# 0kam/alproj

Hardware: AMD Instinct MI355X
Metric: Gpoints/s projected (pinhole + Brown-Conrady, single pose) over the 100M-vertex DSM; CMA-ES iterations/s in `cma` (higher is better)
Workload: dtype f32

## Files before the change

alproj_amd/csrc/alp_cma.hip:

```cpp
#include "alp_points_internal.h"
#include "alp_sampler.h"

#include <cmath>

namespace {

using namespace alp;

constexpr int CMA_MAX_D = SAMPLER_MAX_D;
constexpr int CMA_MAX_P = 4096;
constexpr int CMA_MAX_STARTS = 1024;
constexpr int64_t CMA_MAX_TOTAL = 65536;
constexpr int TELL_THREADS = 256;
constexpr int JACOBI_MAX_SWEEPS = 40;
constexpr double CMA_EPS = 1e-8;
constexpr double CMA_SIGMA_MAX = 1e32;

struct CmaState {
    double mean[CMA_MAX_D], ps[CMA_MAX_D], pc[CMA_MAX_D], d[CMA_MAX_D];
    double C[CMA_MAX_D * CMA_MAX_D], B[CMA_MAX_D * CMA_MAX_D];
    double BD[CMA_MAX_D * CMA_MAX_D];
    double sigma;
    long long g;
    unsigned k0, k1;
};

struct CmaHyper {
    int D, P, mu, dmax, K;
    double mu_eff, c1, cmu, cc, c_sigma, d_sigma, chi_n, cm, sum_w;
};

struct ExpandArgs {
    double tmpl[ALP_NPARAM];
    double lo[CMA_MAX_D], hi[CMA_MAX_D];
    int idx[CMA_MAX_D];
    double origin[3];
};

template <typename T, int DMAX, bool LF>
__global__ __launch_bounds__(256) void cma_generation_kernel(SamplerArgs a0, ExpandArgs e, const CmaState *__restrict__ states, long long P,
                                                             long long total, double *__restrict__ x_out, double *__restrict__ cand_out,
                                                             PoseRec<T> *__restrict__ recs, long long lf_off) {
    const long long cand = ((long long)blockIdx.x * blockDim.x + threadIdx.x) >> 6;
    if (cand >= total) return;
    const long long start = cand / P, draw = cand - start * P;
    const CmaState *st = states + start;
    const int lane = (int)(threadIdx.x & 63);
    SamplerArgs a = a0;
#pragma unroll
    for (int i = 0; i < DMAX; ++i)
        if (i < a.D) a.mean[i] = st->mean[i];
    a.sigma = st->sigma;
    a.gen = (unsigned)st->g;
    a.k0 = st->k0;
    a.k1 = st->k1;
    const double *BD = st->BD;
    double z[DMAX], x[DMAX];
#pragma unroll
    for (int j = 0; j < DMAX; ++j) z[j] = 0.0;
    int accepted = -1;
    for (int base = 0; base < a.n_max && accepted < 0; base += 64) {
        const int t = base + lane;
        bool ok = false;
        if (t < a.n_max) {
            draw_normals<DMAX>(z, a.D, (unsigned)t, (unsigned)draw, a.gen, a.k0, a.k1);
            ok = make_x<DMAX, false>(a, BD, z, x);
        }
        const unsigned long long m = __ballot(ok);
        if (m) accepted = base + __ffsll((long long)m) - 1;
    }
    const int t_final = accepted >= 0 ? accepted : a.n_max;
    if (lane != (t_final & 63)) return;
    draw_normals<DMAX>(z, a.D, (unsigned)t_final, (unsigned)draw, a.gen, a.k0, a.k1);
    make_x<DMAX, true>(a, BD, z, x);
    double prm[ALP_NPARAM];
    for (int k = 0; k < ALP_NPARAM; ++k) prm[k] = e.tmpl[k];
#pragma unroll
    for (int i = 0; i < DMAX; ++i)
        if (i < a.D) {
            double xi = x[i];
            if (accepted < 0 && a.bounded) xi = fmin(fmax(xi, a.lower[i]), a.upper[i]);
            x_out[cand * a.D + i] = xi;
            prm[e.idx[i]] = xi * (e.hi[i] - e.lo[i]) + e.lo[i];
        }
    for (int k = 0; k < ALP_NPARAM; ++k) cand_out[cand * ALP_NPARAM + k] = prm[k];
    double g[POSE_WORDS];
    fold_pose_hd(prm, e.origin, g);
    for (int k = 0; k < POSE_WORDS; ++k) recs[cand].v[k] = (T)g[k];
    if (LF) {
        double lf[POSE_WORDS];
        lens_free_from_general_hd(g, lf);
        for (int k = 0; k < POSE_WORDS; ++k) recs[lf_off + cand].v[k] = (T)lf[k];
    }
}

__device__ __forceinline__ void circle_pair(int m, int r, int k, int *p, int *q) {
    const int a = k == 0 ? m - 1 : (r + k) % (m - 1);
    const int b = (r - k + (m - 1)) % (m - 1);
    *p = a < b ? a : b;
    *q = a < b ? b : a;
}

__device__ void jacobi_eigen(int D, double *C, double *B, double *d2, double *A, double *A2, double *V, double *V2, double *self_,
                             double *oth, double *dlt, int *partner, int *rotated, int *nrot) {
    const int tid = threadIdx.x;
    const int DD = D * D;
    for (int e = tid; e < DD; e += blockDim.x) {
        const int i = e / D, j = e % D;
        double s = 0;
        for (int k = 0; k < D; ++k) s += B[k * D + i] * B[k * D + j];
        A2[e] = s;
    }
    __syncthreads();
    for (int e = tid; e < DD; e += blockDim.x) {
        const int i = e / D, j = e % D;
        double s = 0;
        for (int k = 0; k < D; ++k) s += B[i * D + k] * ((k == j ? 1.5 : 0.0) - 0.5 * A2[k * D + j]);
        V2[e] = s;
    }
    __syncthreads();
    for (int e = tid; e < DD; e += blockDim.x) B[e] = V2[e];
    __syncthreads();
    for (int e = tid; e < DD; e += blockDim.x) {
        const int i = e / D, j = e % D;
        double s = 0;
        for (int k = 0; k < D; ++k) s += C[i * D + k] * B[k * D + j];
        A2[e] = s;
    }
    __syncthreads();
    for (int e = tid; e < DD; e += blockDim.x) {
        const int i = e / D, j = e % D;
        if (i <= j) {
            double s = 0;
            for (int k = 0; k < D; ++k) s += B[k * D + i] * A2[k * D + j];
            A[i * D + j] = s;
            A[j * D + i] = s;
        }
        V[e] = i == j ? 1.0 : 0.0;
    }
    __syncthreads();
    const int m = (D + 1) & ~1;
    for (int sweep = 0; sweep < JACOBI_MAX_SWEEPS && m >= 2; ++sweep) {
        if (tid == 0) *nrot = 0;
        __syncthreads();
        for (int r = 0; r < m - 1; ++r) {
            if (tid < m / 2) {
                int p, q;
                circle_pair(m, r, tid, &p, &q);
                if (q < D) {
                    const double app = A[p * D + p], aqq = A[q * D + q], apq = A[p * D + q];
                    const double g = 100.0 * fabs(apq);
                    double c = 1.0, s = 0.0, t = 0.0;
                    const bool rot = apq != 0.0 && !(fabs(app) + g == fabs(app) && fabs(aqq) + g == fabs(aqq));
                    if (rot) {
                        const double theta = (aqq - app) / (2.0 * apq);
                        if (fabs(theta) > 1e150) t = 0.5 / theta;
                        else {
                            t = 1.0 / (fabs(theta) + sqrt(theta * theta + 1.0));
                            if (theta < 0) t = -t;
                        }
                        c = 1.0 / sqrt(t * t + 1.0);
                        s = t * c;
                        *nrot = 1;
                    }
                    partner[p] = q; partner[q] = p;
                    self_[p] = c; self_[q] = c;
                    oth[p] = -s; oth[q] = s;
                    dlt[p] = -t * apq; dlt[q] = t * apq;
                    rotated[p] = rotated[q] = rot;
                } else if (p < D) {
                    partner[p] = p; self_[p] = 1.0; oth[p] = 0.0; dlt[p] = 0.0; rotated[p] = 0;
                }
            }
            __syncthreads();
            for (int e = tid; e < DD; e += blockDim.x) {
                const int i = e / D, j = e % D;
                double v;
                if (i == j) v = A[e] + dlt[i];
                else if (partner[i] == j && rotated[i]) v = 0.0;
                else {
                    const int lo = i < j ? i : j, hi = i < j ? j : i;
                    const int plo = partner[lo], phi = partner[hi];
                    v = self_[hi] * A[lo * D + hi];
                    if (oth[hi] != 0.0) v += oth[hi] * A[lo * D + phi];
                    v *= self_[lo];
                    if (oth[lo] != 0.0) {
                        double w = self_[hi] * A[plo * D + hi];
                        if (oth[hi] != 0.0) w += oth[hi] * A[plo * D + phi];
                        v += oth[lo] * w;
                    }
                }
                A2[e] = v;
                double u = V[i * D + j] * self_[j];
                if (oth[j] != 0.0) u += V[i * D + partner[j]] * oth[j];
                V2[e] = u;
            }
            __syncthreads();
            for (int e = tid; e < DD; e += blockDim.x) {
                A[e] = A2[e];
                V[e] = V2[e];
            }
            __syncthreads();
        }
        if (*nrot == 0) break;
        __syncthreads();
    }
    for (int e = tid; e < DD; e += blockDim.x) {
        const int i = e / D, j = e % D;
        double s = 0;
        for (int k = 0; k < D; ++k) s += B[i * D + k] * V[k * D + j];
        V2[e] = s;
    }
    for (int i = tid; i < D; i += blockDim.x) d2[i] = A[i * D + i];
    __syncthreads();
    for (int e = tid; e < DD; e += blockDim.x) B[e] = V2[e];
    __syncthreads();
}

template <bool TELL>
__global__ __launch_bounds__(TELL_THREADS) void cma_tell_kernel(CmaHyper h, CmaState *__restrict__ states, const double *__restrict__ weights,
                                                                const double *__restrict__ X_all, const double *__restrict__ sums_all,
                                                                const double *__restrict__ vals_all, double *__restrict__ loss_all,
                                                                int *__restrict__ order_all, double *__restrict__ ys_all,
                                                                double *__restrict__ wio_all) {
    const long long k = blockIdx.x, kP = k * h.P, kPD = kP * h.D;
    CmaState *__restrict__ st = states + k;
    const double *__restrict__ X = X_all + kPD;
    const double *__restrict__ sums = sums_all ? sums_all + kP : nullptr;
    const double n_total = sums_all ? sums_all[(long long)h.K * h.P] : 0.0;
    const double *__restrict__ vals = vals_all ? vals_all + kP : nullptr;
    double *__restrict__ loss_out = loss_all + kP;
    int *__restrict__ order_out = order_all + kP;
    double *__restrict__ ys = ys_all + kPD;
    double *__restrict__ wio = wio_all + kP;
    constexpr int M = CMA_MAX_D * CMA_MAX_D;
    __shared__ double C[M], B[M], A[M], A2[M], V[M], V2[M];
    __shared__ double mean[CMA_MAX_D], d[CMA_MAX_D], yw[CMA_MAX_D], ps[CMA_MAX_D], pc[CMA_MAX_D], d2[CMA_MAX_D];
    __shared__ double self_[CMA_MAX_D], oth[CMA_MAX_D], dlt[CMA_MAX_D];
    __shared__ int partner[CMA_MAX_D], rotated[CMA_MAX_D];
    __shared__ int nrot;
    __shared__ double sig, hsig;
    const int tid = threadIdx.x, D = h.D, P = h.P, DD = D * D;
    for (int e = tid; e < DD; e += blockDim.x) {
        C[e] = st->C[e];
        B[e] = st->B[e];
    }
    for (int i = tid; i < D; i += blockDim.x) {
        mean[i] = st->mean[i];
        d[i] = st->d[i];
        ps[i] = st->ps[i];
        pc[i] = st->pc[i];
    }
    if (tid == 0) sig = st->sigma;
    __syncthreads();
    if (TELL) {
        const long long g = st->g + 1;
        for (int i = tid; i < P; i += blockDim.x) loss_out[i] = vals ? vals[i] : sums[i] / n_total;
        __syncthreads();
        for (int i = tid; i < P; i += blockDim.x) {
            double ki = loss_out[i];
            if (ki != ki) ki = INFINITY;
            int r = 0;
            for (int j = 0; j < P; ++j) {
                double kj = loss_out[j];
                if (kj != kj) kj = INFINITY;
                r += (kj < ki) || (kj == ki && j < i);
            }
            order_out[r] = i;
        }
        __syncthreads();
        const double sigma = sig;
        for (int e = tid; e < P * D; e += blockDim.x) {
            const int r = e / D, j = e % D;
            ys[e] = (X[(long long)order_out[r] * D + j] - mean[j]) / sigma;
        }
        __syncthreads();
        for (int j = tid; j < D; j += blockDim.x) {
            double s = 0.0;
            for (int r = 0; r < h.mu; ++r) s = s + ys[(long long)r * D + j] * weights[r];
            yw[j] = s;
        }
        __syncthreads();
        const double cs = h.c_sigma, cmsig = h.cm * sigma;
        for (int e = tid; e < DD; e += blockDim.x) {
            const int i = e / D, j = e % D;
            double s = 0.0;
            for (int k = 0; k < D; ++k) s += (B[i * D + k] / d[k]) * B[j * D + k];
            A[e] = s;
        }
        for (int j = tid; j < D; j += blockDim.x) mean[j] = mean[j] + cmsig * yw[j];
        __syncthreads();
        const double sq_ps = sqrt(cs * (2.0 - cs) * h.mu_eff);
        for (int i = tid; i < D; i += blockDim.x) {
            double s = 0.0;
            for (int k = 0; k < D; ++k) s += A[i * D + k] * yw[k];
            ps[i] = (1.0 - cs) * ps[i] + sq_ps * s;
        }
        __syncthreads();
        if (tid == 0) {
            double nn = 0.0;
            for (int k = 0; k < D; ++k) nn += ps[k] * ps[k];
            const double norm_ps = sqrt(nn);
            double s2 = sig * exp((cs / h.d_sigma) * (norm_ps / h.chi_n - 1.0));
            sig = s2 < CMA_SIGMA_MAX ? s2 : CMA_SIGMA_MAX;
            const double h_left = norm_ps / sqrt(1.0 - pow(1.0 - cs, (double)(2 * (g + 1))));
            const double h_right = (1.4 + 2.0 / (double)(D + 1)) * h.chi_n;
            hsig = h_left < h_right ? 1.0 : 0.0;
        }
        __syncthreads();
        const double h_sigma = hsig, cc = h.cc;
        const double sq_pc = h_sigma * sqrt(cc * (2.0 - cc) * h.mu_eff);
        for (int i = tid; i < D; i += blockDim.x) pc[i] = (1.0 - cc) * pc[i] + sq_pc * yw[i];
        for (int r = tid; r < P; r += blockDim.x) {
            const double wr = weights[r];
            if (wr >= 0) {
                wio[r] = wr * 1.0;
            } else {
                double nn = 0.0;
                for (int i = 0; i < D; ++i) {
                    double s = 0.0;
                    for (int k = 0; k < D; ++k) s += ys[(long long)r * D + k] * A[i * D + k];
                    nn += s * s;
                }
                const double nrm = sqrt(nn);
                wio[r] = wr * ((double)D / (nrm * nrm + CMA_EPS));
            }
        }
        __syncthreads();
        const double delta_h = (1.0 - h_sigma) * cc * (2.0 - cc);
        const double c1 = h.c1, cmu = h.cmu;
        const double coef = 1.0 + c1 * delta_h - c1 - cmu * h.sum_w;
        for (int e = tid; e < DD; e += blockDim.x) {
            const int i = e / D, j = e % D;
            double rmu = 0.0;
            for (int r = 0; r < P; ++r) rmu += (ys[(long long)r * D + i] * wio[r]) * ys[(long long)r * D + j];
            A2[e] = coef * C[e] + c1 * (pc[i] * pc[j]) + cmu * rmu;
        }
        __syncthreads();
        for (int e = tid; e < DD; e += blockDim.x) C[e] = A2[e];
        if (tid == 0) st->g = g;
        __syncthreads();
    }
    for (int e = tid; e < DD; e += blockDim.x) {
        const int i = e / D, j = e % D;
        A2[e] = (C[i * D + j] + C[j * D + i]) / 2.0;
    }
    __syncthreads();
    for (int e = tid; e < DD; e += blockDim.x) C[e] = A2[e];
    __syncthreads();
    jacobi_eigen(D, C, B, d2, A, A2, V, V2, self_, oth, dlt, partner, rotated, &nrot);
    for (int i = tid; i < D; i += blockDim.x) d[i] = sqrt(d2[i] < 0 ? CMA_EPS : d2[i]);
    __syncthreads();
    for (int e = tid; e < DD; e += blockDim.x) {
        const int i = e / D, j = e % D;
        double s = 0.0;
        for (int k = 0; k < D; ++k) s += (B[i * D + k] * (d[k] * d[k])) * B[j * D + k];
        st->C[e] = s;
        st->B[e] = B[e];
    }
    for (int e = tid; e < h.dmax * h.dmax; e += blockDim.x) {
        const int i = e / h.dmax, j = e % h.dmax;
        st->BD[e] = (i < D && j < D) ? B[i * D + j] * d[j] : 0.0;
    }
    for (int i = tid; i < D; i += blockDim.x) {
        st->d[i] = d[i];
        if (TELL) {
            st->mean[i] = mean[i];
            st->ps[i] = ps[i];
            st->pc[i] = pc[i];
        }
    }
    if (TELL && tid == 0) st->sigma = sig;
}

}

struct alp_cma {
    alp_points *pts = nullptr;
    CmaHyper hy{};
    SamplerArgs sa{};
    ExpandArgs ex{};
    std::vector<uint64_t> seeds;
    bool lens_free = false, shared_pose = false;
    DeviceBuffer<> dev;
    CmaState *st = nullptr;
    double *w = nullptr, *X = nullptr, *cand = nullptr, *loss = nullptr, *ys = nullptr, *wio = nullptr, *vals = nullptr;
    int *order = nullptr;
    bool pending = false;
    bool have_last = false;
    int64_t rows() const { return (int64_t)hy.K * hy.P; }
};

namespace alp {
void cma_points_gone(alp_cma_t *h) { h->pts = nullptr; }
}

namespace {

void fill_state(const alp_cma *h, int k, CmaState *s, const double *mean, double sigma, const double *C, const double *ps, const double *pc,
                int64_t g) {
    const int D = h->hy.D;
    memset(s, 0, sizeof(*s));
    for (int i = 0; i < D; ++i) {
        s->mean[i] = mean[i];
        s->ps[i] = ps[i];
        s->pc[i] = pc[i];
        s->d[i] = 1.0;
        s->B[i * D + i] = 1.0;
    }
    for (int e = 0; e < D * D; ++e) s->C[e] = C[e];
    s->sigma = sigma;
    s->g = g;
    s->k0 = (unsigned)h->seeds[(size_t)k];
    s->k1 = (unsigned)(h->seeds[(size_t)k] >> 32);
}

int upload_states(alp_cma *h, int k0, int n, const CmaState *s) {
    hipStream_t st = ctx().stream;
    ALP_HIP(hipMemcpyAsync(h->st + k0, s, (size_t)n * sizeof(CmaState), hipMemcpyHostToDevice, st));
    hipLaunchKernelGGL(cma_tell_kernel<false>, dim3(n), dim3(TELL_THREADS), 0, st, h->hy, h->st + k0, (const double *)h->w,
                       (const double *)h->X, (const double *)nullptr, (const double *)nullptr, h->loss, h->order, h->ys, h->wio);
    ALP_HIP(hipGetLastError());
    ALP_HIP(hipStreamSynchronize(st));
    return ALP_OK;
}

int usable(alp_cma *h, const char *what) {
    if (int rc = require_init()) return rc;
    if (!h) return fail(ALP_EINVAL, "%s: handle is NULL", what);
    if (h->pending) return fail(ALP_ESTATE, "%s: generations are enqueued; call alp_cma_wait first", what);
    return ALP_OK;
}

template <typename T, int DMAX>
void launch_generation(alp_cma *h, unsigned grid, hipStream_t st) {
    alp_points *p = h->pts;
    PoseRec<T> *recs = (PoseRec<T> *)p->cand_dev;
    if (h->lens_free)
        hipLaunchKernelGGL((cma_generation_kernel<T, DMAX, true>), dim3(grid), dim3(256), 0, st, h->sa, h->ex, (const CmaState *)h->st,
                           (long long)h->hy.P, (long long)h->rows(), h->X, h->cand, recs, (long long)p->cand_cap);
    else
        hipLaunchKernelGGL((cma_generation_kernel<T, DMAX, false>), dim3(grid), dim3(256), 0, st, h->sa, h->ex, (const CmaState *)h->st,
                           (long long)h->hy.P, (long long)h->rows(), h->X, h->cand, recs, (long long)p->cand_cap);
}

template <typename T>
void launch_generation_t(alp_cma *h, unsigned grid, hipStream_t st) {
    if (h->hy.dmax == 12) launch_generation<T, 12>(h, grid, st);
    else if (h->hy.dmax == 24) launch_generation<T, 24>(h, grid, st);
    else launch_generation<T, 32>(h, grid, st);
}

}

extern "C" {

int alp_cma_create_starts(alp_points_t *pts, const double tmpl[ALP_NPARAM], const int32_t *target_idx, int D, const double *lower,
                          const double *upper, int64_t P, int K, const double *weights, const double hyper[ALP_CMA_NHYPER],
                          int n_max_resampling, const uint64_t *seeds, alp_cma_t **out) {
    if (int rc = require_init()) return rc;
    ALP_REQUIRE(out, "out is NULL");
    *out = nullptr;
    ALP_REQUIRE(pts && tmpl && target_idx && lower && upper && weights && hyper && seeds, "NULL argument");
    ALP_REQUIRE(D >= 1 && D <= CMA_MAX_D, "D must be in [1, 32]");
    ALP_REQUIRE(P >= 1 && P <= CMA_MAX_P, "P must be in [1, 4096]");
    ALP_REQUIRE(K >= 1 && K <= CMA_MAX_STARTS, "K must be in [1, 1024]");
    ALP_REQUIRE((int64_t)K * P <= CMA_MAX_TOTAL, "K * P must be at most 65536");
    ALP_REQUIRE(n_max_resampling >= 0 && n_max_resampling <= (1 << 20), "n_max_resampling out of range");
    if (!pts->uo) return fail(ALP_ESTATE, "alp_cma_create: observed uv not set");
    for (int i = 0; i < D; ++i) {
        ALP_REQUIRE(target_idx[i] >= 0 && target_idx[i] < ALP_NPARAM, "target index out of range");
        ALP_REQUIRE(target_idx[i] != 21 && target_idx[i] != 22, "w and h cannot be targets (every candidate must share the image size)");
    }
    const int mu = (int)hyper[0];
    ALP_REQUIRE(mu >= 0 && mu <= P, "mu out of range");
    alp_cma *h = new alp_cma();
    h->pts = pts;
    const int dmax = D <= 12 ? 12 : (D <= 24 ? 24 : 32);
    h->hy = CmaHyper{D, (int)P, mu, dmax, K, hyper[1], hyper[2], hyper[3], hyper[4], hyper[5], hyper[6], hyper[7], hyper[8], hyper[9]};
    h->seeds.assign(seeds, seeds + K);
    memset(&h->sa, 0, sizeof(h->sa));
    for (int i = 0; i < D; ++i) {
        h->sa.lower[i] = 0.0;
        h->sa.upper[i] = 1.0;
    }
    h->sa.D = D;
    h->sa.n_max = n_max_resampling;
    h->sa.bounded = 1;
    memset(&h->ex, 0, sizeof(h->ex));
    for (int k = 0; k < ALP_NPARAM; ++k) h->ex.tmpl[k] = tmpl[k];
    for (int i = 0; i < D; ++i) {
        h->ex.idx[i] = target_idx[i];
        h->ex.lo[i] = lower[i];
        h->ex.hi[i] = upper[i];
    }
    memcpy(h->ex.origin, pts->origin, sizeof(h->ex.origin));
    bool lf = !getenv("ALP_POP_NO_LENS_FREE");
    for (int k = 9; k <= 20 && lf; ++k) lf = tmpl[k] == 0.0;
    for (int i = 0; i < D && lf; ++i) lf = !(target_idx[i] >= 9 && target_idx[i] <= 20);
    bool shared = P > 1 && !lf;
    for (int i = 0; i < D && shared; ++i) shared = target_idx[i] >= 7 && target_idx[i] <= 20;
    h->lens_free = lf;
    h->shared_pose = shared;
    const int64_t R = (int64_t)K * P;
    const size_t sz_state = round_up((int64_t)K * sizeof(CmaState), 256), sz_w = round_up(P * 8, 256), sz_p = round_up(R * 8, 256),
                 sz_pd = round_up(R * D * 8, 256), sz_cand = round_up(R * ALP_NPARAM * 8, 256), sz_ord = round_up(R * 4, 256);
    int rc = h->dev.reserve(sz_state + sz_w + 3 * sz_p + 2 * sz_pd + sz_cand + sz_ord);
    if (!rc) {
        char *q = (char *)h->dev;
        h->st = (CmaState *)q; q += sz_state;
        h->w = (double *)q; q += sz_w;
        h->loss = (double *)q; q += sz_p;
        h->wio = (double *)q; q += sz_p;
        h->vals = (double *)q; q += sz_p;
        h->X = (double *)q; q += sz_pd;
        h->ys = (double *)q; q += sz_pd;
        h->cand = (double *)q; q += sz_cand;
        h->order = (int *)q;
        if (hipMemcpy(h->w, weights, (size_t)P * 8, hipMemcpyHostToDevice) != hipSuccess) rc = fail(ALP_EHIP, "alp_cma_create: weights upload failed");
    }
    if (!rc) rc = points_pop_reserve(pts, R);
    if (!rc) {
        std::vector<double> mean(D, 0.5), C((size_t)D * D, 0.0), zero(D, 0.0);
        for (int i = 0; i < D; ++i) C[(size_t)i * D + i] = 1.0;
        std::vector<CmaState> s((size_t)K);
        for (int k = 0; k < K; ++k) fill_state(h, k, &s[(size_t)k], mean.data(), 1.0, C.data(), zero.data(), zero.data(), 0);
        rc = upload_states(h, 0, K, s.data());
    }
    if (rc) {
        delete h;
        return rc;
    }
    pts->loops.push_back(h);
    *out = h;
    return ALP_OK;
}

int alp_cma_create(alp_points_t *pts, const double tmpl[ALP_NPARAM], const int32_t *target_idx, int D, const double *lower,
                   const double *upper, int64_t P, const double *weights, const double hyper[ALP_CMA_NHYPER], int n_max_resampling,
                   uint64_t seed, alp_cma_t **out) {
    return alp_cma_create_starts(pts, tmpl, target_idx, D, lower, upper, P, 1, weights, hyper, n_max_resampling, &seed, out);
}

int alp_cma_destroy(alp_cma_t *h) {
    if (!h) return ALP_OK;
    if (ctx().ready) hipStreamSynchronize(ctx().stream);
    if (h->pts) {
        h->pts->loop_pending = false;
        auto &v = h->pts->loops;
        for (size_t i = 0; i < v.size(); ++i)
            if (v[i] == h) {
                v.erase(v.begin() + (long)i);
                break;
            }
    }
    delete h;
    return ALP_OK;
}

int alp_cma_set_state_at(alp_cma_t *h, int k, const double *mean, double sigma, const double *C, const double *p_sigma, const double *pc,
                         int64_t generation) {
    if (int rc = usable(h, "alp_cma_set_state")) return rc;
    ALP_REQUIRE(k >= 0 && k < h->hy.K, "start index out of range");
    ALP_REQUIRE(mean && C && p_sigma && pc, "NULL argument");
    ALP_REQUIRE(sigma > 0, "sigma must be positive");
    ALP_REQUIRE(generation >= 0, "generation is negative");
    CmaState s;
    fill_state(h, k, &s, mean, sigma, C, p_sigma, pc, generation);
    return upload_states(h, k, 1, &s);
}

int alp_cma_set_state(alp_cma_t *h, const double *mean, double sigma, const double *C, const double *p_sigma, const double *pc,
                      int64_t generation) {
    return alp_cma_set_state_at(h, 0, mean, sigma, C, p_sigma, pc, generation);
}

int alp_cma_get_state_at(alp_cma_t *h, int k, double *mean, double *sigma, double *C, double *p_sigma, double *pc, int64_t *generation,
                         double *B, double *Dvec) {
    if (int rc = usable(h, "alp_cma_get_state")) return rc;
    ALP_REQUIRE(k >= 0 && k < h->hy.K, "start index out of range");
    CmaState s;
    ALP_HIP(hipMemcpyAsync(&s, h->st + k, sizeof(s), hipMemcpyDeviceToHost, ctx().stream));
    ALP_HIP(hipStreamSynchronize(ctx().stream));
    const int D = h->hy.D;
    for (int i = 0; i < D; ++i) {
        if (mean) mean[i] = s.mean[i];
        if (p_sigma) p_sigma[i] = s.ps[i];
        if (pc) pc[i] = s.pc[i];
        if (Dvec) Dvec[i] = s.d[i];
    }
    for (int e = 0; e < D * D; ++e) {
        if (C) C[e] = s.C[e];
        if (B) B[e] = s.B[e];
    }
    if (sigma) *sigma = s.sigma;
    if (generation) *generation = s.g;
    return ALP_OK;
}

int alp_cma_get_state(alp_cma_t *h, double *mean, double *sigma, double *C, double *p_sigma, double *pc, int64_t *generation, double *B,
                      double *Dvec) {
    return alp_cma_get_state_at(h, 0, mean, sigma, C, p_sigma, pc, generation, B, Dvec);
}

int alp_cma_run(alp_cma_t *h, int64_t generations, int loss_kind, double f_scale) {
    if (int rc = usable(h, "alp_cma_run")) return rc;
    ALP_REQUIRE(generations >= 0, "generations is negative");
    ALP_REQUIRE(loss_kind == ALP_LOSS_MEAN_DIST || loss_kind == ALP_LOSS_HUBER, "unknown loss_kind");
    alp_points *p = h->pts;
    if (!p) return fail(ALP_ESTATE, "alp_cma_run: the point set of this device loop has been destroyed");
    if (p->pending_P > 0 || p->loop_pending)
        return fail(ALP_ESTATE, "alp_cma_run: the point set has an evaluation enqueued that has not been waited for");
    if (generations == 0) return ALP_OK;
    const int64_t R = h->rows();
    if (int rc = points_pop_reserve(p, R)) return rc;
    const unsigned grid = (unsigned)((R * 64 + 255) / 256);
    const bool batched = h->hy.K > 1;
    hipStream_t st = ctx().stream;
    h->pending = true;
    p->loop_pending = true;
    for (int64_t g = 0; g < generations; ++g) {
        if (p->precision == ALP_F64) launch_generation_t<double>(h, grid, st);
        else launch_generation_t<float>(h, grid, st);
        ALP_HIP(hipGetLastError());
        if (int rc = popeval_launch(p, R, loss_kind, f_scale, h->lens_free, h->shared_pose, batched, h->cand)) return rc;
        hipLaunchKernelGGL(cma_tell_kernel<true>, dim3(h->hy.K), dim3(TELL_THREADS), 0, st, h->hy, h->st, (const double *)h->w,
                           (const double *)h->X, (const double *)p->sums_dev, (const double *)nullptr, h->loss, h->order, h->ys, h->wio);
        ALP_HIP(hipGetLastError());
    }
    h->have_last = true;
    return ALP_OK;
}

int alp_cma_wait(alp_cma_t *h) {
    if (int rc = require_init()) return rc;
    ALP_REQUIRE(h, "handle is NULL");
    if (!h->pending) return fail(ALP_ESTATE, "alp_cma_wait: nothing enqueued");
    h->pending = false;
    if (h->pts) h->pts->loop_pending = false;
    ALP_HIP(hipStreamSynchronize(ctx().stream));
    return ALP_OK;
}

int alp_cma_tell_host(alp_cma_t *h, const double *X, const double *losses, int32_t *order_out) {
    if (int rc = usable(h, "alp_cma_tell_host")) return rc;
    ALP_REQUIRE(X && losses, "NULL argument");
    const int64_t R = h->rows(), D = h->hy.D;
    hipStream_t st = ctx().stream;
    ALP_HIP(hipMemcpyAsync(h->X, X, (size_t)(R * D) * 8, hipMemcpyHostToDevice, st));
    ALP_HIP(hipMemcpyAsync(h->vals, losses, (size_t)R * 8, hipMemcpyHostToDevice, st));
    hipLaunchKernelGGL(cma_tell_kernel<true>, dim3(h->hy.K), dim3(TELL_THREADS), 0, st, h->hy, h->st, (const double *)h->w,
                       (const double *)h->X, (const double *)nullptr, (const double *)h->vals, h->loss, h->order, h->ys, h->wio);
    ALP_HIP(hipGetLastError());
    if (order_out) ALP_HIP(hipMemcpyAsync(order_out, h->order, (size_t)R * 4, hipMemcpyDeviceToHost, st));
    ALP_HIP(hipStreamSynchronize(st));
    h->have_last = false;
    return ALP_OK;
}

int alp_cma_fetch_last(alp_cma_t *h, double *X, double *cand, double *losses) {
    if (int rc = usable(h, "alp_cma_fetch_last")) return rc;
    if (!h->have_last) return fail(ALP_ESTATE, "alp_cma_fetch_last: no device generation has run");
    const int64_t R = h->rows(), D = h->hy.D;
    hipStream_t st = ctx().stream;
    if (X) ALP_HIP(hipMemcpyAsync(X, h->X, (size_t)(R * D) * 8, hipMemcpyDeviceToHost, st));
    if (cand) ALP_HIP(hipMemcpyAsync(cand, h->cand, (size_t)R * ALP_NPARAM * 8, hipMemcpyDeviceToHost, st));
    if (losses) ALP_HIP(hipMemcpyAsync(losses, h->loss, (size_t)R * 8, hipMemcpyDeviceToHost, st));
    ALP_HIP(hipStreamSynchronize(st));
    return ALP_OK;
}

}
```

alproj_amd/csrc/host/alp_fold.h:

```cpp
#pragma once

#include <cmath>

#include "alproj_hip.h"

#if defined(__HIP__)
#define ALP_HD __host__ __device__
#else
#define ALP_HD
#endif

namespace alp {

ALP_HD inline double fold_sin(double a) { return std::sin(a); }
ALP_HD inline double fold_cos(double a) { return std::cos(a); }
ALP_HD inline double fold_tan(double a) { return std::tan(a); }

template <typename T>
ALP_HD inline void fold_pose_any(const T p[ALP_NPARAM], double w, double h, const double origin[3], T rec[POSE_WORDS]) {
    const T X = p[0], Y = p[1], Z = p[2], fov = p[3], pan_d = p[4], tilt_d = p[5],
            roll_d = p[6];
    const T cx = p[23], cy = p[24];
    const double pi = M_PI;

    const T fov_x = fov * pi / 180;
    const T fov_y = fov_x * h / w;
    const T fx = w / (2 * fold_tan(fov_x / 2));
    const T fy = h / (2 * fold_tan(fov_y / 2));

    const T a = pan_d * pi / 180;
    const T b = -(tilt_d + 90) * pi / 180;
    const T c = -roll_d * pi / 180;
    const T rz[3][3] = {{fold_cos(a), -fold_sin(a), 0}, {fold_sin(a), fold_cos(a), 0}, {0, 0, 1}};
    const T rx[3][3] = {{1, 0, 0}, {0, fold_cos(b), -fold_sin(b)}, {0, fold_sin(b), fold_cos(b)}};
    const T ry[3][3] = {{fold_cos(c), 0, fold_sin(c)}, {0, 1, 0}, {-fold_sin(c), 0, fold_cos(c)}};
    T rxy[3][3], R[3][3];
    for (int i = 0; i < 3; ++i)
        for (int j = 0; j < 3; ++j) {
            T s = 0;
            for (int k = 0; k < 3; ++k) s += rx[i][k] * ry[k][j];
            rxy[i][j] = s;
        }
    for (int i = 0; i < 3; ++i)
        for (int j = 0; j < 3; ++j) {
            T s = 0;
            for (int k = 0; k < 3; ++k) s += rxy[i][k] * rz[k][j];
            R[i][j] = s;
        }
    const T d[3] = {origin[0] - X, origin[1] - Y, origin[2] - Z};
    T row[3][4];
    for (int i = 0; i < 3; ++i) {
        for (int j = 0; j < 3; ++j) row[i][j] = R[i][j];
        row[i][3] = R[i][0] * d[0] + R[i][1] * d[1] + R[i][2] * d[2];
    }
    const double c0 = (double)(float)((w - 1) / 2);
    const double c1 = (double)(float)((h - 1) / 2);
    const double A = (w - c0) / c0;
    for (int j = 0; j < 4; ++j) {
        const T rowx = fx * row[0][j] + cx * row[2][j];
        const T rowy = fy * row[1][j] + cy * row[2][j];
        rec[0 + j] = A * row[2][j] - rowx / c0;
        rec[4 + j] = rowy / c1 - row[2][j];
        rec[8 + j] = row[2][j];
    }
    for (int i = 0; i < 6; ++i) rec[12 + i] = p[9 + i];
    rec[18] = 1 + p[7];
    rec[19] = 1 + p[8];
    rec[20] = 2 * p[15];
    rec[21] = 2 * p[16];
    for (int i = 0; i < 4; ++i) rec[22 + i] = p[17 + i];
    rec[26] = c0;
    rec[27] = c1;
    rec[28] = -c0;
    rec[29] = -c1;
    rec[30] = rec[31] = 0;
}

ALP_HD inline void fold_pose_hd(const double p[ALP_NPARAM], const double origin[3], double rec[POSE_WORDS]) {
    fold_pose_any<double>(p, p[21], p[22], origin, rec);
}

ALP_HD inline void lens_free_from_general_hd(const double g[POSE_WORDS], double rec[POSE_WORDS]) {
    const double sy = g[18] / g[19];
    for (int i = 0; i < POSE_WORDS; ++i) rec[i] = 0;
    for (int j = 0; j < 4; ++j) {
        rec[0 + j] = g[28] * g[0 + j];
        rec[4 + j] = (g[29] * sy) * g[4 + j];
        rec[8 + j] = g[8 + j];
    }
    rec[26] = g[26];
    rec[27] = g[27];
}

}
```

Measured before the change: 498.4.

## Parallelize CMA ask/tell: wave-spread trig, per-wave Jacobi rounds, shared-memory small tell

The ask kernel keeps the accepted sample in every lane so it is not redrawn, and spreads the eight pose trig evaluations across lanes with shuffles. The Jacobi eigen solver replaces the block barrier and copy-back with per-wave round buffers, ping-pong buffer swaps and a ballot to detect convergence, and the modulo work in pair selection is removed. A SMALL tell variant stages losses, weights, order and ys in shared memory, and the block size now scales with the problem size. This targets the many serial double-precision steps and barriers per CMA iteration, at the cost of more register pressure and more complex code paths.

```diff
diff --git a/alproj_amd/csrc/alp_cma.hip b/alproj_amd/csrc/alp_cma.hip
--- a/alproj_amd/csrc/alp_cma.hip
+++ b/alproj_amd/csrc/alp_cma.hip
@@ -12,6 +12,7 @@
 constexpr int CMA_MAX_STARTS = 1024;
 constexpr int64_t CMA_MAX_TOTAL = 65536;
 constexpr int TELL_THREADS = 256;
+constexpr int TELL_SMALL_P = 256;
 constexpr int JACOBI_MAX_SWEEPS = 40;
 constexpr double CMA_EPS = 1e-8;
 constexpr double CMA_SIGMA_MAX = 1e32;
@@ -57,22 +58,25 @@
     const double *BD = st->BD;
     double z[DMAX], x[DMAX];
 #pragma unroll
-    for (int j = 0; j < DMAX; ++j) z[j] = 0.0;
+    for (int j = 0; j < DMAX; ++j) z[j] = x[j] = 0.0;
     int accepted = -1;
+    constexpr bool KEEP = DMAX <= 24;
     for (int base = 0; base < a.n_max && accepted < 0; base += 64) {
         const int t = base + lane;
         bool ok = false;
         if (t < a.n_max) {
             draw_normals<DMAX>(z, a.D, (unsigned)t, (unsigned)draw, a.gen, a.k0, a.k1);
-            ok = make_x<DMAX, false>(a, BD, z, x);
+            ok = make_x<DMAX, KEEP>(a, BD, z, x);
         }
         const unsigned long long m = __ballot(ok);
         if (m) accepted = base + __ffsll((long long)m) - 1;
     }
     const int t_final = accepted >= 0 ? accepted : a.n_max;
-    if (lane != (t_final & 63)) return;
-    draw_normals<DMAX>(z, a.D, (unsigned)t_final, (unsigned)draw, a.gen, a.k0, a.k1);
-    make_x<DMAX, true>(a, BD, z, x);
+    const int src = t_final & 63;
+    if ((!KEEP || accepted < 0) && lane == src) {
+        draw_normals<DMAX>(z, a.D, (unsigned)t_final, (unsigned)draw, a.gen, a.k0, a.k1);
+        make_x<DMAX, true>(a, BD, z, x);
+    }
     double prm[ALP_NPARAM];
     for (int k = 0; k < ALP_NPARAM; ++k) prm[k] = e.tmpl[k];
 #pragma unroll
@@ -80,12 +84,29 @@
         if (i < a.D) {
             double xi = x[i];
             if (accepted < 0 && a.bounded) xi = fmin(fmax(xi, a.lower[i]), a.upper[i]);
-            x_out[cand * a.D + i] = xi;
+            if (lane == src) x_out[cand * a.D + i] = xi;
             prm[e.idx[i]] = xi * (e.hi[i] - e.lo[i]) + e.lo[i];
         }
+    double ang[FOLD_ANGLES];
+    FoldTrigValues<double> tr;
+    fold_angles<double>(prm, prm[21], prm[22], ang);
+    double mine = 0.0;
+#pragma unroll
+    for (int k = 0; k < FOLD_ANGLES; ++k) {
+        const double ak = __shfl(ang[k], src);
+        if (fold_trig_angle(lane & 7) == k) mine = ak;
+    }
+    double val = 0.0;
+    if (lane < FOLD_SIN_A) {
+        if (lane < FOLD_COS_A) val = fold_tan(mine);
+        else val = fold_cos(mine);
+    } else if (lane < FOLD_TRIGS) val = fold_sin(mine);
+#pragma unroll
+    for (int v = 0; v < FOLD_TRIGS; ++v) tr.v[v] = __shfl(val, v);
+    if (lane != src) return;
     for (int k = 0; k < ALP_NPARAM; ++k) cand_out[cand * ALP_NPARAM + k] = prm[k];
     double g[POSE_WORDS];
-    fold_pose_hd(prm, e.origin, g);
+    fold_pose_with<double>(prm, prm[21], prm[22], e.origin, tr, g);
     for (int k = 0; k < POSE_WORDS; ++k) recs[cand].v[k] = (T)g[k];
     if (LF) {
         double lf[POSE_WORDS];
@@ -95,43 +116,51 @@
 }
 
 __device__ __forceinline__ void circle_pair(int m, int r, int k, int *p, int *q) {
-    const int a = k == 0 ? m - 1 : (r + k) % (m - 1);
-    const int b = (r - k + (m - 1)) % (m - 1);
+    const int a = k == 0 ? m - 1 : (r + k >= m - 1 ? r + k - (m - 1) : r + k);
+    const int b = r - k < 0 ? r - k + (m - 1) : r - k;
     *p = a < b ? a : b;
     *q = a < b ? b : a;
 }
 
-__device__ void jacobi_eigen(int D, double *C, double *B, double *d2, double *A, double *A2, double *V, double *V2, double *self_,
-                             double *oth, double *dlt, int *partner, int *rotated, int *nrot) {
-    const int tid = threadIdx.x;
+struct JacobiRound {
+    double self_[CMA_MAX_D], oth[CMA_MAX_D], dlt[CMA_MAX_D];
+    int partner[CMA_MAX_D], rotated[CMA_MAX_D];
+};
+
+__device__ void jacobi_eigen(int D, double *C, double *B, double *d2, double *A, double *A2, double *V, double *V2, JacobiRound *rnd) {
+    const int tid = threadIdx.x, nthr = blockDim.x;
     const int DD = D * D;
-    for (int e = tid; e < DD; e += blockDim.x) {
+    for (int e = tid; e < DD; e += nthr) {
         const int i = e / D, j = e % D;
         double s = 0;
+#pragma unroll 4
         for (int k = 0; k < D; ++k) s += B[k * D + i] * B[k * D + j];
         A2[e] = s;
     }
     __syncthreads();
-    for (int e = tid; e < DD; e += blockDim.x) {
+    for (int e = tid; e < DD; e += nthr) {
         const int i = e / D, j = e % D;
         double s = 0;
+#pragma unroll 4
         for (int k = 0; k < D; ++k) s += B[i * D + k] * ((k == j ? 1.5 : 0.0) - 0.5 * A2[k * D + j]);
         V2[e] = s;
     }
     __syncthreads();
-    for (int e = tid; e < DD; e += blockDim.x) B[e] = V2[e];
-    __syncthreads();
-    for (int e = tid; e < DD; e += blockDim.x) {
+    for (int e = tid; e < DD; e += nthr) B[e] = V2[e];
+    __syncthreads();
+    for (int e = tid; e < DD; e += nthr) {
         const int i = e / D, j = e % D;
         double s = 0;
+#pragma unroll 4
         for (int k = 0; k < D; ++k) s += C[i * D + k] * B[k * D + j];
         A2[e] = s;
     }
     __syncthreads();
-    for (int e = tid; e < DD; e += blockDim.x) {
+    for (int e = tid; e < DD; e += nthr) {
         const int i = e / D, j = e % D;
         if (i <= j) {
             double s = 0;
+#pragma unroll 4
             for (int k = 0; k < D; ++k) s += B[k * D + i] * A2[k * D + j];
             A[i * D + j] = s;
             A[j * D + i] = s;
@@ -140,13 +169,16 @@
     }
     __syncthreads();
     const int m = (D + 1) & ~1;
+    const int lane = tid & 63;
+    JacobiRound &w = rnd[tid >> 6];
+    const int i0 = tid / D, j0 = tid % D, istep = nthr / D, jstep = nthr % D;
     for (int sweep = 0; sweep < JACOBI_MAX_SWEEPS && m >= 2; ++sweep) {
-        if (tid == 0) *nrot = 0;
-        __syncthreads();
+        int any = 0;
         for (int r = 0; r < m - 1; ++r) {
-            if (tid < m / 2) {
+            int rot_here = 0;
+            if (lane < m / 2) {
                 int p, q;
-                circle_pair(m, r, tid, &p, &q);
+                circle_pair(m, r, lane, &p, &q);
                 if (q < D) {
                     const double app = A[p * D + p], aqq = A[q * D + q], apq = A[p * D + q];
                     const double g = 100.0 * fabs(apq);
@@ -161,63 +193,64 @@
                         }
                         c = 1.0 / sqrt(t * t + 1.0);
                         s = t * c;
-                        *nrot = 1;
+                        rot_here = 1;
                     }
-                    partner[p] = q; partner[q] = p;
-                    self_[p] = c; self_[q] = c;
-                    oth[p] = -s; oth[q] = s;
-                    dlt[p] = -t * apq; dlt[q] = t * apq;
-                    rotated[p] = rotated[q] = rot;
+                    w.partner[p] = q; w.partner[q] = p;
+                    w.self_[p] = c; w.self_[q] = c;
+                    w.oth[p] = -s; w.oth[q] = s;
+                    w.dlt[p] = -t * apq; w.dlt[q] = t * apq;
+                    w.rotated[p] = w.rotated[q] = rot;
                 } else if (p < D) {
-                    partner[p] = p; self_[p] = 1.0; oth[p] = 0.0; dlt[p] = 0.0; rotated[p] = 0;
+                    w.partner[p] = p; w.self_[p] = 1.0; w.oth[p] = 0.0; w.dlt[p] = 0.0; w.rotated[p] = 0;
                 }
             }
+            __builtin_amdgcn_wave_barrier();
+            int i = i0, j = j0;
+            for (int e = tid; e < DD; e += nthr) {
+                const int pi = w.partner[i], pj = w.partner[j], roti = w.rotated[i];
+                const double ci = w.self_[i], cj = w.self_[j], oi = w.oth[i], oj = w.oth[j], di = w.dlt[i];
+                const bool up = i < j;
+                const int lo = up ? i : j, hi = up ? j : i, plo = up ? pi : pj, phi = up ? pj : pi;
+                const double clo = up ? ci : cj, chi = up ? cj : ci, olo = up ? oi : oj, ohi = up ? oj : oi;
+                const double a_e = A[e], a_lh = A[lo * D + hi], a_lp = A[lo * D + phi], a_ph = A[plo * D + hi], a_pp = A[plo * D + phi];
+                const double v_ij = V[i * D + j], v_ip = V[i * D + pj];
+                double v = chi * a_lh;
+                v = ohi != 0.0 ? v + ohi * a_lp : v;
+                v *= clo;
+                double t = chi * a_ph;
+                t = ohi != 0.0 ? t + ohi * a_pp : t;
+                v = olo != 0.0 ? v + olo * t : v;
+                v = (pi == j && roti) ? 0.0 : v;
+                v = i == j ? a_e + di : v;
+                A2[e] = v;
+                double u = v_ij * cj;
+                u = oj != 0.0 ? u + v_ip * oj : u;
+                V2[e] = u;
+                i += istep;
+                j += jstep;
+                if (j >= D) { j -= D; ++i; }
+            }
+            any |= __ballot(rot_here) != 0;
             __syncthreads();
-            for (int e = tid; e < DD; e += blockDim.x) {
-                const int i = e / D, j = e % D;
-                double v;
-                if (i == j) v = A[e] + dlt[i];
-                else if (partner[i] == j && rotated[i]) v = 0.0;
-                else {
-                    const int lo = i < j ? i : j, hi = i < j ? j : i;
-                    const int plo = partner[lo], phi = partner[hi];
-                    v = self_[hi] * A[lo * D + hi];
-                    if (oth[hi] != 0.0) v += oth[hi] * A[lo * D + phi];
-                    v *= self_[lo];
-                    if (oth[lo] != 0.0) {
-                        double w = self_[hi] * A[plo * D + hi];
-                        if (oth[hi] != 0.0) w += oth[hi] * A[plo * D + phi];
-                        v += oth[lo] * w;
-                    }
-                }
-                A2[e] = v;
-                double u = V[i * D + j] * self_[j];
-                if (oth[j] != 0.0) u += V[i * D + partner[j]] * oth[j];
-                V2[e] = u;
-            }
-            __syncthreads();
-            for (int e = tid; e < DD; e += blockDim.x) {
-                A[e] = A2[e];
-                V[e] = V2[e];
-            }
-            __syncthreads();
-        }
-        if (*nrot == 0) break;
-        __syncthreads();
-    }
-    for (int e = tid; e < DD; e += blockDim.x) {
+            double *sw = A; A = A2; A2 = sw;
+            sw = V; V = V2; V2 = sw;
+        }
+        if (!any) break;
+    }
+    for (int e = tid; e < DD; e += nthr) {
         const int i = e / D, j = e % D;
         double s = 0;
+#pragma unroll 4
         for (int k = 0; k < D; ++k) s += B[i * D + k] * V[k * D + j];
         V2[e] = s;
     }
-    for (int i = tid; i < D; i += blockDim.x) d2[i] = A[i * D + i];
-    __syncthreads();
-    for (int e = tid; e < DD; e += blockDim.x) B[e] = V2[e];
-    __syncthreads();
-}
-
-template <bool TELL>
+    for (int i = tid; i < D; i += nthr) d2[i] = A[i * D + i];
+    __syncthreads();
+    for (int e = tid; e < DD; e += nthr) B[e] = V2[e];
+    __syncthreads();
+}
+
+template <bool TELL, bool SMALL = false>
 __global__ __launch_bounds__(TELL_THREADS) void cma_tell_kernel(CmaHyper h, CmaState *__restrict__ states, const double *__restrict__ weights,
                                                                 const double *__restrict__ X_all, const double *__restrict__ sums_all,
                                                                 const double *__restrict__ vals_all, double *__restrict__ loss_all,
@@ -231,14 +264,15 @@
     const double *__restrict__ vals = vals_all ? vals_all + kP : nullptr;
     double *__restrict__ loss_out = loss_all + kP;
     int *__restrict__ order_out = order_all + kP;
-    double *__restrict__ ys = ys_all + kPD;
-    double *__restrict__ wio = wio_all + kP;
     constexpr int M = CMA_MAX_D * CMA_MAX_D;
     __shared__ double C[M], B[M], A[M], A2[M], V[M], V2[M];
+    double *const ys = SMALL ? V : ys_all + kPD;
+    double *const loss = SMALL ? V2 : loss_out;
+    double *const wio = SMALL ? V2 + TELL_SMALL_P : wio_all + kP;
+    const double *const wts = SMALL ? V2 + 2 * TELL_SMALL_P : weights;
+    int *const order = SMALL ? (int *)(V2 + 3 * TELL_SMALL_P) : order_out;
     __shared__ double mean[CMA_MAX_D], d[CMA_MAX_D], yw[CMA_MAX_D], ps[CMA_MAX_D], pc[CMA_MAX_D], d2[CMA_MAX_D];
-    __shared__ double self_[CMA_MAX_D], oth[CMA_MAX_D], dlt[CMA_MAX_D];
-    __shared__ int partner[CMA_MAX_D], rotated[CMA_MAX_D];
-    __shared__ int nrot;
+    __shared__ JacobiRound rnd[TELL_THREADS / 64];
     __shared__ double sig, hsig;
     const int tid = threadIdx.x, D = h.D, P = h.P, DD = D * D;
     for (int e = tid; e < DD; e += blockDim.x) {
@@ -255,29 +289,39 @@
     __syncthreads();
     if (TELL) {
         const long long g = st->g + 1;
-        for (int i = tid; i < P; i += blockDim.x) loss_out[i] = vals ? vals[i] : sums[i] / n_total;
-        __syncthreads();
         for (int i = tid; i < P; i += blockDim.x) {
-            double ki = loss_out[i];
+            const double l = vals ? vals[i] : sums[i] / n_total;
+            loss_out[i] = l;
+            if (SMALL) {
+                loss[i] = l;
+                V2[2 * TELL_SMALL_P + i] = weights[i];
+            }
+        }
+        __syncthreads();
+        for (int i = tid; i < P; i += blockDim.x) {
+            double ki = loss[i];
             if (ki != ki) ki = INFINITY;
             int r = 0;
+#pragma unroll 4
             for (int j = 0; j < P; ++j) {
-                double kj = loss_out[j];
+                double kj = loss[j];
                 if (kj != kj) kj = INFINITY;
                 r += (kj < ki) || (kj == ki && j < i);
             }
             order_out[r] = i;
+            if (SMALL) order[r] = i;
         }
         __syncthreads();
         const double sigma = sig;
         for (int e = tid; e < P * D; e += blockDim.x) {
             const int r = e / D, j = e % D;
-            ys[e] = (X[(long long)order_out[r] * D + j] - mean[j]) / sigma;
+            ys[e] = (X[(long long)order[r] * D + j] - mean[j]) / sigma;
         }
         __syncthreads();
         for (int j = tid; j < D; j += blockDim.x) {
             double s = 0.0;
-            for (int r = 0; r < h.mu; ++r) s = s + ys[(long long)r * D + j] * weights[r];
+#pragma unroll 4
+            for (int r = 0; r < h.mu; ++r) s = s + ys[(long long)r * D + j] * wts[r];
             yw[j] = s;
         }
         __syncthreads();
@@ -285,6 +329,7 @@
         for (int e = tid; e < DD; e += blockDim.x) {
             const int i = e / D, j = e % D;
             double s = 0.0;
+#pragma unroll 4
             for (int k = 0; k < D; ++k) s += (B[i * D + k] / d[k]) * B[j * D + k];
             A[e] = s;
         }
@@ -293,6 +338,7 @@
         const double sq_ps = sqrt(cs * (2.0 - cs) * h.mu_eff);
         for (int i = tid; i < D; i += blockDim.x) {
             double s = 0.0;
+#pragma unroll 4
             for (int k = 0; k < D; ++k) s += A[i * D + k] * yw[k];
             ps[i] = (1.0 - cs) * ps[i] + sq_ps * s;
         }
@@ -312,13 +358,14 @@
         const double sq_pc = h_sigma * sqrt(cc * (2.0 - cc) * h.mu_eff);
         for (int i = tid; i < D; i += blockDim.x) pc[i] = (1.0 - cc) * pc[i] + sq_pc * yw[i];
         for (int r = tid; r < P; r += blockDim.x) {
-            const double wr = weights[r];
+            const double wr = wts[r];
             if (wr >= 0) {
                 wio[r] = wr * 1.0;
             } else {
                 double nn = 0.0;
                 for (int i = 0; i < D; ++i) {
                     double s = 0.0;
+#pragma unroll 4
                     for (int k = 0; k < D; ++k) s += ys[(long long)r * D + k] * A[i * D + k];
                     nn += s * s;
                 }
@@ -333,6 +380,7 @@
         for (int e = tid; e < DD; e += blockDim.x) {
             const int i = e / D, j = e % D;
             double rmu = 0.0;
+#pragma unroll 4
             for (int r = 0; r < P; ++r) rmu += (ys[(long long)r * D + i] * wio[r]) * ys[(long long)r * D + j];
             A2[e] = coef * C[e] + c1 * (pc[i] * pc[j]) + cmu * rmu;
         }
@@ -348,12 +396,13 @@
     __syncthreads();
     for (int e = tid; e < DD; e += blockDim.x) C[e] = A2[e];
     __syncthreads();
-    jacobi_eigen(D, C, B, d2, A, A2, V, V2, self_, oth, dlt, partner, rotated, &nrot);
+    jacobi_eigen(D, C, B, d2, A, A2, V, V2, rnd);
     for (int i = tid; i < D; i += blockDim.x) d[i] = sqrt(d2[i] < 0 ? CMA_EPS : d2[i]);
     __syncthreads();
     for (int e = tid; e < DD; e += blockDim.x) {
         const int i = e / D, j = e % D;
         double s = 0.0;
+#pragma unroll 4
         for (int k = 0; k < D; ++k) s += (B[i * D + k] * (d[k] * d[k])) * B[j * D + k];
         st->C[e] = s;
         st->B[e] = B[e];
@@ -371,6 +420,20 @@
         }
     }
     if (TELL && tid == 0) st->sigma = sig;
+}
+
+int tell_threads(const CmaHyper &h) {
+    const int want = h.D * h.D > h.P ? h.D * h.D : h.P;
+    const int waves = (want + 63) / 64;
+    return 64 * (waves < 1 ? 1 : waves > TELL_THREADS / 64 ? TELL_THREADS / 64 : waves);
+}
+
+bool tell_small(const CmaHyper &h) { return h.P <= TELL_SMALL_P && h.P * h.D <= CMA_MAX_D * CMA_MAX_D; }
+
+template <typename... Args>
+void launch_tell(const CmaHyper &hy, hipStream_t st, Args... args) {
+    if (tell_small(hy)) hipLaunchKernelGGL((cma_tell_kernel<true, true>), dim3(hy.K), dim3(tell_threads(hy)), 0, st, hy, args...);
+    else hipLaunchKernelGGL((cma_tell_kernel<true, false>), dim3(hy.K), dim3(tell_threads(hy)), 0, st, hy, args...);
 }
 
 }
@@ -418,7 +481,7 @@
 int upload_states(alp_cma *h, int k0, int n, const CmaState *s) {
     hipStream_t st = ctx().stream;
     ALP_HIP(hipMemcpyAsync(h->st + k0, s, (size_t)n * sizeof(CmaState), hipMemcpyHostToDevice, st));
-    hipLaunchKernelGGL(cma_tell_kernel<false>, dim3(n), dim3(TELL_THREADS), 0, st, h->hy, h->st + k0, (const double *)h->w,
+    hipLaunchKernelGGL(cma_tell_kernel<false>, dim3(n), dim3(tell_threads(h->hy)), 0, st, h->hy, h->st + k0, (const double *)h->w,
                        (const double *)h->X, (const double *)nullptr, (const double *)nullptr, h->loss, h->order, h->ys, h->wio);
     ALP_HIP(hipGetLastError());
     ALP_HIP(hipStreamSynchronize(st));
@@ -624,8 +687,8 @@
         else launch_generation_t<float>(h, grid, st);
         ALP_HIP(hipGetLastError());
         if (int rc = popeval_launch(p, R, loss_kind, f_scale, h->lens_free, h->shared_pose, batched, h->cand)) return rc;
-        hipLaunchKernelGGL(cma_tell_kernel<true>, dim3(h->hy.K), dim3(TELL_THREADS), 0, st, h->hy, h->st, (const double *)h->w,
-                           (const double *)h->X, (const double *)p->sums_dev, (const double *)nullptr, h->loss, h->order, h->ys, h->wio);
+        launch_tell(h->hy, st, h->st, (const double *)h->w, (const double *)h->X, (const double *)p->sums_dev, (const double *)nullptr,
+                    h->loss, h->order, h->ys, h->wio);
         ALP_HIP(hipGetLastError());
     }
     h->have_last = true;
@@ -649,8 +712,8 @@
     hipStream_t st = ctx().stream;
     ALP_HIP(hipMemcpyAsync(h->X, X, (size_t)(R * D) * 8, hipMemcpyHostToDevice, st));
     ALP_HIP(hipMemcpyAsync(h->vals, losses, (size_t)R * 8, hipMemcpyHostToDevice, st));
-    hipLaunchKernelGGL(cma_tell_kernel<true>, dim3(h->hy.K), dim3(TELL_THREADS), 0, st, h->hy, h->st, (const double *)h->w,
-                       (const double *)h->X, (const double *)nullptr, (const double *)h->vals, h->loss, h->order, h->ys, h->wio);
+    launch_tell(h->hy, st, h->st, (const double *)h->w, (const double *)h->X, (const double *)nullptr, (const double *)h->vals, h->loss,
+                h->order, h->ys, h->wio);
     ALP_HIP(hipGetLastError());
     if (order_out) ALP_HIP(hipMemcpyAsync(order_out, h->order, (size_t)R * 4, hipMemcpyDeviceToHost, st));
     ALP_HIP(hipStreamSynchronize(st));
diff --git a/alproj_amd/csrc/host/alp_fold.h b/alproj_amd/csrc/host/alp_fold.h
--- a/alproj_amd/csrc/host/alp_fold.h
+++ b/alproj_amd/csrc/host/alp_fold.h
@@ -16,24 +16,60 @@
 ALP_HD inline double fold_cos(double a) { return std::cos(a); }
 ALP_HD inline double fold_tan(double a) { return std::tan(a); }
 
+enum { FOLD_ANGLES = 5, FOLD_TRIGS = 8 };
+enum { FOLD_TAN_X = 0, FOLD_TAN_Y = 1, FOLD_COS_A = 2, FOLD_COS_B = 3, FOLD_COS_C = 4, FOLD_SIN_A = 5, FOLD_SIN_B = 6, FOLD_SIN_C = 7 };
+ALP_HD inline int fold_trig_angle(int v) { return v < 5 ? v : v - 3; }
+
 template <typename T>
-ALP_HD inline void fold_pose_any(const T p[ALP_NPARAM], double w, double h, const double origin[3], T rec[POSE_WORDS]) {
-    const T X = p[0], Y = p[1], Z = p[2], fov = p[3], pan_d = p[4], tilt_d = p[5],
-            roll_d = p[6];
-    const T cx = p[23], cy = p[24];
+ALP_HD inline void fold_angles(const T p[ALP_NPARAM], double w, double h, T ang[FOLD_ANGLES]) {
+    const T fov = p[3], pan_d = p[4], tilt_d = p[5], roll_d = p[6];
     const double pi = M_PI;
-
     const T fov_x = fov * pi / 180;
     const T fov_y = fov_x * h / w;
-    const T fx = w / (2 * fold_tan(fov_x / 2));
-    const T fy = h / (2 * fold_tan(fov_y / 2));
+    ang[0] = fov_x / 2;
+    ang[1] = fov_y / 2;
+    ang[2] = pan_d * pi / 180;
+    ang[3] = -(tilt_d + 90) * pi / 180;
+    ang[4] = -roll_d * pi / 180;
+}
 
-    const T a = pan_d * pi / 180;
-    const T b = -(tilt_d + 90) * pi / 180;
-    const T c = -roll_d * pi / 180;
-    const T rz[3][3] = {{fold_cos(a), -fold_sin(a), 0}, {fold_sin(a), fold_cos(a), 0}, {0, 0, 1}};
-    const T rx[3][3] = {{1, 0, 0}, {0, fold_cos(b), -fold_sin(b)}, {0, fold_sin(b), fold_cos(b)}};
-    const T ry[3][3] = {{fold_cos(c), 0, fold_sin(c)}, {0, 1, 0}, {-fold_sin(c), 0, fold_cos(c)}};
+template <typename T>
+struct FoldTrigCalls {
+    T ang[FOLD_ANGLES];
+    ALP_HD T tan_x() const { return fold_tan(ang[0]); }
+    ALP_HD T tan_y() const { return fold_tan(ang[1]); }
+    ALP_HD T cos_a() const { return fold_cos(ang[2]); }
+    ALP_HD T sin_a() const { return fold_sin(ang[2]); }
+    ALP_HD T cos_b() const { return fold_cos(ang[3]); }
+    ALP_HD T sin_b() const { return fold_sin(ang[3]); }
+    ALP_HD T cos_c() const { return fold_cos(ang[4]); }
+    ALP_HD T sin_c() const { return fold_sin(ang[4]); }
+};
+
+template <typename T>
+struct FoldTrigValues {
+    T v[FOLD_TRIGS];
+    ALP_HD T tan_x() const { return v[FOLD_TAN_X]; }
+    ALP_HD T tan_y() const { return v[FOLD_TAN_Y]; }
+    ALP_HD T cos_a() const { return v[FOLD_COS_A]; }
+    ALP_HD T sin_a() const { return v[FOLD_SIN_A]; }
+    ALP_HD T cos_b() const { return v[FOLD_COS_B]; }
+    ALP_HD T sin_b() const { return v[FOLD_SIN_B]; }
+    ALP_HD T cos_c() const { return v[FOLD_COS_C]; }
+    ALP_HD T sin_c() const { return v[FOLD_SIN_C]; }
+};
+
+template <typename T, typename Trig>
+ALP_HD inline void fold_pose_with(const T p[ALP_NPARAM], double w, double h, const double origin[3], const Trig &tg, T rec[POSE_WORDS]) {
+    const T X = p[0], Y = p[1], Z = p[2];
+    const T cx = p[23], cy = p[24];
+
+    const T fx = w / (2 * tg.tan_x());
+    const T fy = h / (2 * tg.tan_y());
+
+    const T rz[3][3] = {{tg.cos_a(), -tg.sin_a(), 0}, {tg.sin_a(), tg.cos_a(), 0}, {0, 0, 1}};
+    const T rx[3][3] = {{1, 0, 0}, {0, tg.cos_b(), -tg.sin_b()}, {0, tg.sin_b(), tg.cos_b()}};
+    const T ry[3][3] = {{tg.cos_c(), 0, tg.sin_c()}, {0, 1, 0}, {-tg.sin_c(), 0, tg.cos_c()}};
     T rxy[3][3], R[3][3];
     for (int i = 0; i < 3; ++i)
         for (int j = 0; j < 3; ++j) {
@@ -76,6 +112,13 @@
     rec[30] = rec[31] = 0;
 }
 
+template <typename T>
+ALP_HD inline void fold_pose_any(const T p[ALP_NPARAM], double w, double h, const double origin[3], T rec[POSE_WORDS]) {
+    FoldTrigCalls<T> tg;
+    fold_angles<T>(p, w, h, tg.ang);
+    fold_pose_with<T>(p, w, h, origin, tg, rec);
+}
+
 ALP_HD inline void fold_pose_hd(const double p[ALP_NPARAM], const double origin[3], double rec[POSE_WORDS]) {
     fold_pose_any<double>(p, p[21], p[22], origin, rec);
 }
```

Result: no change. 500.5, median of 2 (+0.4%).
